# ggerganov/ggml

Measured on AMD Instinct MI355X. Metric: effective TFLOPS (2*M*N*K), Q4_K mul_mat [4096x4096]x[4096x512], higher is better.
Workload: dtype f16; 1 GPU; Q4_K MUL_MAT [4096x4096]·[4096x512] per GPU; step = Q8_K activation quantize + fp16-MFMA GEMM, W and fp32 X resident in HBM; M_per_gpu=4096, K=4096, B=512, parallelism=row-split x1, output left sharded, gemm_variant=0, splitk=0

## Files before the change

### ggml_amd/csrc/gemm_kq_t64.inc

```
#include "epilogue.h"
#include "quantize_dev.h"
template <int TYPE, int TM, bool IDS = false, int ABL = 0, bool TAIL = false, bool FQ = false>
__global__ __launch_bounds__(512) void k_gemm_kq_t64(const gemm_params p) {
    static_assert(TYPE == CDNA4_Q4_K || TYPE == CDNA4_Q4_0R, "k_gemm_kq_t64: Q4_K, and Q4_0 as its resident Q4_0R image");
    static_assert(!(FQ && TYPE != CDNA4_Q4_K), "the one-launch step quantizes to Q8_K: Q4_K only");
    static_assert(TM == 128 || TM == 256, "tile rows");
    static_assert(!(FQ && IDS), "the one-launch step is the plain MUL_MAT's");
    constexpr int TB = 128, NST = 3, BNF = 4;
    constexpr int MG = TM / 64, KW = 8 / MG;
    constexpr int NKK = 8 / KW;
    constexpr int NSB = KW == 4 ? 1 : 2;
    constexpr int RS = 256, XS = TB * RS;
    constexpr int WRS = 64, WS = TM * WRS;
    constexpr int ST = XS + WS;
    constexpr int XL = XS / 1024 / 4;
    constexpr int WL = WS / 1024 / 4;
    constexpr int NL = XL + WL;
    constexpr int BLK = QT<TYPE>::BYTES;
    constexpr int HB = TM * 16;
    constexpr int HR = TM / 4;
    constexpr int RING = NST * ST > 128 * 1024 ? NST * ST : 128 * 1024;
    constexpr int abl = ABL;
    constexpr int TRB = (ABL & 256) ? 8 * 16 * 4 * 4 : 0;
    constexpr int SMEM = RING + 2 * HB + TRB;
    static_assert(SMEM <= 160 * 1024, "LDS budget");
    __shared__ __attribute__((aligned(16))) uint8_t smem[SMEM];
    __shared__ int xchg_failed;

    const int tid = threadIdx.x, lane = tid & 63, j = lane & 31, h = lane >> 5;
    const int wave = __builtin_amdgcn_readfirstlane(tid >> 6);
    const int mg = wave % MG, kq = wave / MG;
    const int nblk = gridDim.x;
    int L = blockIdx.x;
    if ((nblk & 7) == 0 && !(IDS && p.tile_order != nullptr)) L = (blockIdx.x & 7) * (nblk >> 3) + (blockIdx.x >> 3);
    int tile_b = L % p.tiles_b, ks, tile_m;
    [[maybe_unused]] int nfrag = BNF;
    if (IDS && p.tile_order != nullptr) {
        tile_b = p.tile_order[L / p.tiles_m]; tile_m = L % p.tiles_m; ks = 0;
        nfrag = p.tile_nfrag[tile_b];
    } else { L /= p.tiles_b; ks = L % p.splitk; tile_m = L / p.splitk; }
    const int m0 = tile_m * TM, b0 = tile_b * TB;
    int64_t wexp = 0;
    if constexpr (IDS) {
        const int e = p.tile_expert[tile_b];
        if (e < 0) return;
        wexp = (int64_t)e * p.w_expert_bytes;
    }
    const int nsb_all = p.K / 256;
    int nsb, sb0;
    const bool deep = p.splitk > 2 || (p.splitk == 2 && (p.tune & 2));
    if (deep) { const int base = nsb_all / p.splitk, rem = nsb_all % p.splitk; nsb = base + (ks < rem ? 1 : 0); sb0 = ks * base + min(ks, rem); }
    else { nsb = p.partial ? (ks == 0 ? p.sb_split : nsb_all - p.sb_split) : nsb_all; sb0 = p.partial ? (ks == 0 ? 0 : p.sb_split) : 0; }
    const int nstage = nsb * 2;
    const uint32_t lds0 = CDNA4_LDS_BASE(smem);
    const bool traced = (ABL & 256) && p.trace != nullptr && blockIdx.x == 0;
    if (traced && tid == 0) { p.trace[0] = __builtin_amdgcn_s_memtime(); p.trace[1] = __builtin_amdgcn_s_memrealtime(); }
    auto mile = [&](int idx) __attribute__((always_inline)) {
        if constexpr ((ABL & 256) != 0) { if (traced && tid == 0) p.trace[idx] = __builtin_amdgcn_s_memrealtime(); }
    };
    auto stamp = [&](int s_, int ph) __attribute__((always_inline)) {
        if constexpr ((ABL & 256) != 0) {
            if (traced && s_ >= 16 && s_ < 32) {
                const uint32_t t = (uint32_t)__builtin_amdgcn_s_memtime();
                if (lane == 0) *reinterpret_cast<uint32_t *>(smem + RING + 2 * HB + ((wave * 16 + (s_ - 16)) * 4 + ph) * 4) = t;
            }
        }
    };

    floatx16 acc[2][BNF];
#pragma unroll
    for (int mb = 0; mb < 2; mb++)
#pragma unroll
        for (int i = 0; i < BNF; i++)
#pragma unroll
            for (int r = 0; r < 16; r++) acc[mb][i][r] = 0.f;

    const bool loader = wave < 4;
    uint32_t xvoff0, wvoff[WL];
    { const int pc = (wave & 3) * 64 + lane, row = pc >> 4, c = (pc & 15) ^ (row & 15); xvoff0 = (uint32_t)row * 256u + c * 16; }
#pragma unroll
    for (int i = 0; i < WL; i++) {
        const int pc = ((wave & 3) + 4 * i) * 64 + lane, row = pc >> 2, c = (pc & 3) ^ ((row >> 2) & 3);
        wvoff[i] = (uint32_t)(min(m0 + row, p.M - 1) - m0) * (uint32_t)p.w_row_bytes + c * 16;
    }
    const char *const xbase = (const char *)p.xh + ((int64_t)sb0 * 2 * p.B + b0) * 256;
    const char *const wbase = (const char *)p.W + wexp + (int64_t)m0 * p.w_row_bytes + (int64_t)sb0 * BLK + 16;
    auto issue_piece = [&](int i, int st, int slot) __attribute__((always_inline)) {
        const uint32_t l = lds0 + slot * ST;
        if (i < XL) {
            if (!(abl & 1)) {
                if constexpr (FQ) CDNA4_DMA16_SC1(xvoff0, xbase + (int64_t)st * p.B * 256 + i * 4096, l + ((wave & 3) + 4 * i) * 1024);
                else CDNA4_DMA16(xvoff0, xbase + (int64_t)st * p.B * 256 + i * 4096, l + ((wave & 3) + 4 * i) * 1024);
            }
        }
        else if (!(abl & 2)) CDNA4_DMA16(wvoff[i - XL], wbase + (int64_t)(st >> 1) * BLK + (st & 1) * 64, l + XS + ((wave & 3) + 4 * (i - XL)) * 1024);
    };
    auto issue = [&](int st, int slot) __attribute__((always_inline)) {
#pragma unroll
        for (int i = 0; i < NL; i++) issue_piece(i, st, slot);
    };
    const uint32_t hvoff = (uint32_t)(min(m0 + (wave & 3) * HR + (lane & (HR - 1)), p.M - 1) - m0) * (uint32_t)p.w_row_bytes;
    const char *const hbase = (const char *)p.W + wexp + (int64_t)m0 * p.w_row_bytes + (int64_t)sb0 * BLK;
    auto hissue = [&](int sb) __attribute__((always_inline)) {
        if (!(abl & 2)) CDNA4_DMA16_LANES(hvoff, hbase + (int64_t)sb * BLK, lds0 + RING + (sb & 1) * HB + (wave & 3) * HR * 16, HR);
    };
    auto hread = [&](int sb) __attribute__((always_inline)) { return *reinterpret_cast<const u32x4 *>(smem + RING + (sb & 1) * HB + (mg * 64 + lane) * 16); };

    DqConst dq; dq.init();
    const int gl = KW == 4 ? (kq >> 1) : kq;
    const int hi = KW == 4 ? (kq & 1) : 0;
    const int q3 = 2 * gl + hi;
    uint32_t rmask = hi ? dq.m4c : dq.m4, rmagic = hi ? dq.magic64 : dq.magic;
    const half_t roff_h = hi ? (half_t)-72.f : (half_t)-1032.f;
    const half2_t roff = {roff_h, roff_h};
    const int xswz = j & 15;

    auto sc_pack = [&](const u32x4 &hdr, auto PART, int q) __attribute__((always_inline)) -> uint32_t {
        constexpr int part = decltype(PART)::value;
        if constexpr (TYPE == CDNA4_Q4_0R) {
            const uint32_t w2 = (q >> 1) ? (part ? hdr.w : hdr.y) : (part ? hdr.z : hdr.x);
            return (w2 >> (16u * (uint32_t)(q & 1))) & 0xFFFFu;
        }
        const uint32_t sh8 = 8u * (uint32_t)q;
        uint32_t s6, m6;
        if constexpr (part == 0) { s6 = (hdr.y >> sh8) & 63u; m6 = (hdr.z >> sh8) & 63u; }
        else { s6 = ((hdr.w >> sh8) & 0xFu) | (((hdr.y >> (sh8 + 6)) & 3u) << 4); m6 = ((hdr.w >> (sh8 + 4)) & 0xFu) | (((hdr.z >> (sh8 + 6)) & 3u) << 4); }
        const float d = h2f(hdr.x & 0xFFFF), dmin = h2f(hdr.x >> 16);
        const half_t s = (half_t)(d * (float)s6);
        const half_t c = (half_t)(8.f * (float)s - dmin * (float)m6);
        return __builtin_bit_cast(uint32_t, half2_t{s, c});
    };
    Raw<TYPE> raw[2];
    typename Raw<TYPE>::Sc z[2];
    uint32_t zp[2][NSB];
    half8_t xa[2][BNF];
    uint32_t wf[2][2][4];
    if constexpr ((ABL & 4) != 0) {
#pragma unroll
        for (int i = 0; i < 2 * BNF; i++) { u32x4 zz = {(uint32_t)lane, 1u, 2u, 3u}; asm volatile("" : "+v"(zz)); xa[i / BNF][i % BNF] = __builtin_bit_cast(half8_t, zz); }
    }
    auto read_xa = [&](int slot, int set, int t, auto PF) __attribute__((always_inline)) {
        constexpr bool pf = decltype(PF)::value;
        const uint8_t *xs = smem + slot * ST + j * RS;
        const int ch = KW == 4 ? hi * 4 + 2 * h + t : (t >> 1) * 4 + 2 * h + (t & 1);
        const int coff = ((gl * 8 + ch) ^ xswz) << 4;
        if (abl & 4) return;
#pragma unroll
        for (int bf = 0; bf < BNF; bf++) if (!pf || bf < nfrag) xa[set][bf] = *reinterpret_cast<const half8_t *>(xs + bf * 32 * RS + coff);
    };
    auto read_w = [&](int slot) __attribute__((always_inline)) {
#pragma unroll
        for (int mb = 0; mb < 2; mb++) {
            const int row = mg * 64 + mb * 32 + j;
            raw[mb].q = *reinterpret_cast<const u32x4 *>(smem + slot * ST + XS + row * WRS + (((2 * gl + h) ^ ((row >> 2) & 3)) << 4));
        }
    };
    auto scales_next = [&](const u32x4 &hdr, auto PART) __attribute__((always_inline)) {
#pragma unroll
        for (int i = 0; i < NSB; i++) {
            uint32_t a = sc_pack(hdr, PART, q3 + i), b = a;
            CDNA4_SWAP32(a, b);
            zp[0][i] = a; zp[1][i] = b;
        }
    };
    auto set_z = [&]() __attribute__((always_inline)) {
#pragma unroll
        for (int mb = 0; mb < 2; mb++) {
            const half2_t lo = as_h2(zp[mb][0]);
            z[mb].SL = half2_t{lo.x, lo.x}; z[mb].CL = half2_t{lo.y, lo.y};
            if constexpr (NSB == 2) { const half2_t hh = as_h2(zp[mb][1]); z[mb].SH = half2_t{hh.x, hh.x}; z[mb].CH = half2_t{hh.y, hh.y}; }
        }
    };
    auto pbits = [&](int mb, int t, int i) __attribute__((always_inline)) -> uint32_t {
        if (abl & 8) return raw[mb].q.x;
        if constexpr (KW == 4) {
            const uint32_t src = (i < 2) ? (t ? raw[mb].q.z : raw[mb].q.x) : (t ? raw[mb].q.w : raw[mb].q.y);
            const uint32_t v = (((i & 1) ? src >> 8 : src) & rmask) | rmagic;
            const half2_t r = __builtin_elementwise_fma(as_h2(v) + roff, z[mb].SL, z[mb].CL);
            return __builtin_bit_cast(uint32_t, r);
        } else return raw[mb].pairbits(t, i, z[mb], dq);
    };
    auto mfma8 = [&](int set, auto PF, auto &&between) __attribute__((always_inline)) {
        constexpr bool pf = decltype(PF)::value;
#pragma unroll
        for (int mb = 0; mb < 2; mb++) {
            const u32x4 cw = {wf[set][mb][0], wf[set][mb][1], wf[set][mb][2], wf[set][mb][3]};
            const half8_t wfk = __builtin_bit_cast(half8_t, cw);
#pragma unroll
            for (int bf = 0; bf < BNF; bf++) {
                __builtin_amdgcn_sched_barrier(0);
                if constexpr ((ABL & 32) != 0) asm volatile("" ::"v"(xa[set][bf]), "v"(wfk));
                else if (!pf || bf < nfrag) acc[mb][bf] = __builtin_amdgcn_mfma_f32_32x32x16_f16(xa[set][bf], wfk, acc[mb][bf], 0, 0, 0);
                __builtin_amdgcn_sched_barrier(0);
                between(mb * 4 + bf);
            }
        }
    };
    typedef std::integral_constant<bool, true> yes_t; typedef std::integral_constant<bool, false> no_t;
    typedef std::integral_constant<int, 0> p0_t; typedef std::integral_constant<int, 1> p1_t;

    if constexpr (FQ) {
        const int nsbK = p.K >> 8, units = (p.tune & 8) ? 0 : p.B * nsbK, g16 = tid >> 4, l16 = tid & 15;
        int u = (int)blockIdx.x * 32 + g16;
        float e[16];
        auto load_unit = [&](int uu) __attribute__((always_inline)) {
            const int b = uu / nsbK, sb = uu - b * nsbK;
            const float *px = p.xf + (int64_t)b * p.xf_row + sb * 256 + 8 * l16;
#pragma unroll
            for (int i = 0; i < 4; i++) {
                const float4 v = *reinterpret_cast<const float4 *>(px + 128 * (i >> 1) + 4 * (i & 1));
                e[4 * i] = v.x; e[4 * i + 1] = v.y; e[4 * i + 2] = v.z; e[4 * i + 3] = v.w;
            }
        };
#pragma unroll
        for (int i = 0; i < 16; i++) e[i] = 0.f;
        if (u < units) load_unit(u);
#pragma unroll
        for (int i = 0; i < 16; i++) CDNA4_PIN(e[i]);
        if (loader) {
            hissue(0); hissue(nsb > 1 ? 1 : 0);
#pragma unroll
            for (int i = XL; i < NL; i++) issue_piece(i, 0, 0);
#pragma unroll
            for (int i = XL; i < NL; i++) issue_piece(i, 1, 1);
        }
        {
            __amdgpu_buffer_rsrc_t img = __builtin_amdgcn_make_buffer_rsrc((void *)p.xh, 0, (int)((int64_t)p.B * p.K * 2), 0x00020000);
            while (u < units) {
                const int b = u / nsbK, sb = u - b * nsbK;
                u32x4 o0, o1;
                q8_K_group16_image(e, l16, o0, o1);
                const int off0 = ((2 * sb) * p.B + b) * 256 + 16 * l16;
                __builtin_amdgcn_raw_buffer_store_b128(o0, img, off0, 0, 16);
                __builtin_amdgcn_raw_buffer_store_b128(o1, img, off0 + p.B * 256, 0, 16);
                u += nblk * 32;
                if (u < units) load_unit(u);
            }
        }
        CDNA4_WAIT_VM(0);
        __syncthreads();
        mile(4);
        if (tid == 0) {
            xchg_failed = ((p.tune & 4) || cdna4_grid_barrier(p.gbar, (unsigned)nblk)) ? 0 : 1;
            if (xchg_failed) cdna4_report_fault(p.fault, 1u);
        }
        __syncthreads();
        if (xchg_failed) {
            for (int i = tid; i < TB * TM; i += 512) {
                const int b = b0 + i / TM, m = m0 + i % TM;
                if (b < p.B && m < p.M) p.Y[(int64_t)b * p.y_row + m] = __builtin_nanf("");
            }
            return;
        }
        mile(5);
        if (loader) {
#pragma unroll
            for (int i = 0; i < XL; i++) issue_piece(i, 0, 0);
#pragma unroll
            for (int i = 0; i < XL; i++) issue_piece(i, 1, 1);
            CDNA4_WAIT_VM(XL);
        }
    } else if (loader) {
        hissue(0); hissue(nsb > 1 ? 1 : 0);
        issue(0, 0); issue(1, 1);
        CDNA4_WAIT_VM(NL);
    }
    __builtin_amdgcn_s_barrier();
    asm volatile("" ::: "memory");
    mile(6);
    u32x4 hcur = hread(0);
    read_w(0); read_xa(0, 0, 0, std::integral_constant<bool, false>{});
    scales_next(hcur, p0_t{});
    set_z();
#pragma unroll
    for (int mb = 0; mb < 2; mb++)
#pragma unroll
        for (int i = 0; i < 4; i++) wf[0][mb][i] = pbits(mb, 0, i);
    int slot = 0;
    auto stage = [&](auto LDF, auto PART, auto NXF, auto L2F, auto L3F, auto PF, int s) __attribute__((always_inline)) {
        constexpr int part = decltype(PART)::value;
        constexpr bool ld = decltype(LDF)::value, nx = decltype(NXF)::value, l2 = decltype(L2F)::value, l3 = decltype(L3F)::value;
        constexpr int G = (NKK - 1) * 8;
        const int slot1 = slot == 2 ? 0 : slot + 1, slot2 = slot == 0 ? 2 : slot - 1;
        stamp(s, 0);
        if constexpr (nx && part == 1) hcur = hread((s + 1) >> 1);
#pragma unroll
        for (int t = 0; t + 1 < NKK; t++) {
            read_xa(slot, (t + 1) & 1, t + 1, PF);
            mfma8(t & 1, PF, [&](int i8) __attribute__((always_inline)) {
                wf[(t + 1) & 1][i8 >> 2][i8 & 3] = pbits(i8 >> 2, t + 1, i8 & 3);
                if constexpr (nx) {
                    if (t == 0 && i8 == 2) { if constexpr (part == 0) scales_next(hcur, p1_t{}); else scales_next(hcur, p0_t{}); }
                }
                if constexpr (ld && l2) {
                    const int g = t * 8 + i8;
                    if constexpr (part == 1 && l3) { if (g == 0) hissue((s + 3) >> 1); }
#pragma unroll
                    for (int i = 0; i < NL; i++) if (i * G / NL == g) issue_piece(i, s + 2, slot2);
                }
            });
        }
        if constexpr (nx) {
            stamp(s, 1);
            if constexpr (ld) {
                if constexpr (l2) CDNA4_WAIT_VM(NL + ((part == 1 && l3) ? 1 : 0)); else CDNA4_WAIT_VM(0);
            }
            CDNA4_WAIT_LGKM0();
            stamp(s, 2);
            if (!(abl & 16)) __builtin_amdgcn_s_barrier();
            asm volatile("" ::: "memory");
            stamp(s, 3);
            __builtin_amdgcn_sched_barrier(0);
            read_w(slot1); read_xa(slot1, 0, 0, PF);
            __builtin_amdgcn_sched_barrier(0);
        }
        mfma8((NKK - 1) & 1, PF, [&](int i8) __attribute__((always_inline)) {
            if constexpr (nx) {
                if (i8 == 3) set_z();
                if (i8 >= 4) { const int q = (i8 - 4) * 2; wf[0][q >> 2][q & 3] = pbits(q >> 2, 0, q & 3); wf[0][(q + 1) >> 2][(q + 1) & 3] = pbits((q + 1) >> 2, 0, (q + 1) & 3); }
            }
        });
        slot = slot1;
    };
    auto k_loop = [&](auto LDF, auto PF) __attribute__((always_inline)) {
        int s = 0;
        for (; s + 5 < nstage; s += 2) { stage(LDF, p0_t{}, yes_t{}, yes_t{}, yes_t{}, PF, s); stage(LDF, p1_t{}, yes_t{}, yes_t{}, yes_t{}, PF, s + 1); }
        if (s + 3 < nstage) { stage(LDF, p0_t{}, yes_t{}, yes_t{}, yes_t{}, PF, s); stage(LDF, p1_t{}, yes_t{}, yes_t{}, no_t{}, PF, s + 1); s += 2; }
        stage(LDF, p0_t{}, yes_t{}, no_t{}, no_t{}, PF, s); stage(LDF, p1_t{}, no_t{}, no_t{}, no_t{}, PF, s + 1);
    };
    if constexpr (IDS && TM == 128) {
        if (nfrag < BNF) { if (loader) k_loop(yes_t{}, yes_t{}); else k_loop(no_t{}, yes_t{}); }
        else { if (loader) k_loop(yes_t{}, no_t{}); else k_loop(no_t{}, no_t{}); }
    } else { if (loader) k_loop(yes_t{}, no_t{}); else k_loop(no_t{}, no_t{}); }

    __syncthreads();
    if constexpr ((ABL & 256) != 0) {
        if (traced) {
            if (tid == 0) { p.trace[2] = __builtin_amdgcn_s_memtime(); p.trace[3] = __builtin_amdgcn_s_memrealtime(); }
            reinterpret_cast<uint32_t *>(p.trace + 8)[tid] = reinterpret_cast<const uint32_t *>(smem + RING + 2 * HB)[tid];
        }
    }
    float4 *red = reinterpret_cast<float4 *>(smem);
    const int tile_id = tile_m * p.tiles_b + tile_b;
    bool out_keeper = false; int out_fb0 = 0;
    constexpr bool has_tail = TAIL && !IDS;
    auto finish = [&](auto KQ) __attribute__((always_inline)) {
        constexpr int kqc = decltype(KQ)::value;
        constexpr int H1 = KW / 2;
        constexpr int keep0 = (kqc & H1) ? 2 : 0, send0 = 2 - keep0;
        float4 *mine = red + (size_t)(mg + MG * kqc) * 1024, *theirs = red + (size_t)(mg + MG * (kqc ^ H1)) * 1024;
#pragma unroll
        for (int mb = 0; mb < 2; mb++)
#pragma unroll
            for (int e = 0; e < 2; e++)
#pragma unroll
                for (int q4 = 0; q4 < 4; q4++) {
                    const floatx16 &a = acc[mb][send0 + e];
                    mine[((mb * 2 + e) * 4 + q4) * 64 + lane] = make_float4(a[4 * q4], a[4 * q4 + 1], a[4 * q4 + 2], a[4 * q4 + 3]);
                }
        __syncthreads();
#pragma unroll
        for (int mb = 0; mb < 2; mb++)
#pragma unroll
            for (int e = 0; e < 2; e++)
#pragma unroll
                for (int q4 = 0; q4 < 4; q4++) {
                    const float4 v = theirs[((mb * 2 + e) * 4 + q4) * 64 + lane];
                    floatx16 &a = acc[mb][keep0 + e];
                    a[4 * q4] += v.x; a[4 * q4 + 1] += v.y; a[4 * q4 + 2] += v.z; a[4 * q4 + 3] += v.w;
                }
        constexpr int NBH = KW == 4 ? 1 : 2;
        constexpr int fb0 = KW == 4 ? keep0 + (kqc & 1) : keep0;
        if constexpr (KW == 4) {
            constexpr int give = keep0 + 1 - (kqc & 1);
            float4 *theirs2 = red + (size_t)(mg + MG * (kqc ^ 1)) * 1024;
            __syncthreads();
#pragma unroll
            for (int mb = 0; mb < 2; mb++)
#pragma unroll
                for (int q4 = 0; q4 < 4; q4++) {
                    const floatx16 &a = acc[mb][give];
                    mine[(mb * 4 + q4) * 64 + lane] = make_float4(a[4 * q4], a[4 * q4 + 1], a[4 * q4 + 2], a[4 * q4 + 3]);
                }
            __syncthreads();
#pragma unroll
            for (int mb = 0; mb < 2; mb++)
#pragma unroll
                for (int q4 = 0; q4 < 4; q4++) {
                    const float4 v = theirs2[(mb * 4 + q4) * 64 + lane];
                    floatx16 &a = acc[mb][fb0];
                    a[4 * q4] += v.x; a[4 * q4 + 1] += v.y; a[4 * q4 + 2] += v.z; a[4 * q4 + 3] += v.w;
                }
        }
        bool keeper = true;
        if (TM == 128 && deep) {
            constexpr int WF4 = NBH * 2 * 4 * 64;
            const int S = p.splitk;
            float4 *slots = reinterpret_cast<float4 *>(p.partial) + ((size_t)tile_id * S * 8 + (mg + MG * kqc)) * WF4;
            {
                __amdgpu_buffer_rsrc_t rsrc = __builtin_amdgcn_make_buffer_rsrc(slots + (size_t)ks * 8 * WF4, 0, WF4 * 16, 0x00020000);
#pragma unroll
                for (int e = 0; e < NBH; e++)
#pragma unroll
                    for (int mb = 0; mb < 2; mb++)
#pragma unroll
                        for (int q4 = 0; q4 < 4; q4++) {
                            const floatx16 &a = acc[mb][fb0 + e];
                            const float4 v = make_float4(a[4 * q4], a[4 * q4 + 1], a[4 * q4 + 2], a[4 * q4 + 3]);
                            __builtin_amdgcn_raw_buffer_store_b128(__builtin_bit_cast(u32x4, v), rsrc, (((e * 2 + mb) * 4 + q4) * 64 + lane) * 16, 0, 16);
                        }
                CDNA4_WAIT_VM(0);
            }
            __syncthreads();
            if (tid == 0) {
                unsigned *ticket = p.flags + 8192 + tile_id;
                const unsigned old = __hip_atomic_fetch_add(ticket, 1u, __ATOMIC_RELAXED, __HIP_MEMORY_SCOPE_AGENT);
                xchg_failed = old == (unsigned)(S - 1);
                if (xchg_failed) __hip_atomic_store(ticket, 0u, __ATOMIC_RELAXED, __HIP_MEMORY_SCOPE_AGENT);
            }
            __syncthreads();
            keeper = xchg_failed != 0;
            if (keeper) {
                float4 sum[NBH * 8];
                for (int k2 = 0; k2 < S; k2++) {
                    float4 v[NBH * 8];
                    if (k2 == ks) {
#pragma unroll
                        for (int e = 0; e < NBH; e++)
#pragma unroll
                            for (int mb = 0; mb < 2; mb++)
#pragma unroll
                                for (int q4 = 0; q4 < 4; q4++) { const floatx16 &a = acc[mb][fb0 + e]; v[(e * 2 + mb) * 4 + q4] = make_float4(a[4 * q4], a[4 * q4 + 1], a[4 * q4 + 2], a[4 * q4 + 3]); }
                    } else {
                        __amdgpu_buffer_rsrc_t rin = __builtin_amdgcn_make_buffer_rsrc(slots + (size_t)k2 * 8 * WF4, 0, WF4 * 16, 0x00020000);
#pragma unroll
                        for (int i = 0; i < NBH * 8; i++) v[i] = __builtin_bit_cast(float4, __builtin_amdgcn_raw_buffer_load_b128(rin, (i * 64 + lane) * 16, 0, 17));
                    }
#pragma unroll
                    for (int i = 0; i < NBH * 8; i++) {
                        if (k2 == 0) sum[i] = v[i];
                        else { sum[i].x += v[i].x; sum[i].y += v[i].y; sum[i].z += v[i].z; sum[i].w += v[i].w; }
                    }
                }
#pragma unroll
                for (int e = 0; e < NBH; e++)
#pragma unroll
                    for (int mb = 0; mb < 2; mb++)
#pragma unroll
                        for (int q4 = 0; q4 < 4; q4++) {
                            const float4 v = sum[(e * 2 + mb) * 4 + q4];
                            floatx16 &a = acc[mb][fb0 + e];
                            a[4 * q4] = v.x; a[4 * q4 + 1] = v.y; a[4 * q4 + 2] = v.z; a[4 * q4 + 3] = v.w;
                        }
            }
        } else if (p.partial) {
            mile(266);
            constexpr int WF4 = NBH * 2 * 4 * 64;
            keeper = (fb0 >> 1) == ks;
            float4 *slot_out = reinterpret_cast<float4 *>(p.partial) + ((size_t)(tile_id * 2 + (ks ^ 1)) * 8 + (mg + MG * kqc)) * WF4;
            float4 *slot_in = reinterpret_cast<float4 *>(p.partial) + ((size_t)(tile_id * 2 + ks) * 8 + (mg + MG * kqc)) * WF4;
            const unsigned my_xcc = __builtin_amdgcn_s_getreg(20 | (3 << 11)) & 15u;
            if (!keeper) {
                __amdgpu_buffer_rsrc_t rsrc = __builtin_amdgcn_make_buffer_rsrc(slot_out, 0, WF4 * 16, 0x00020000);
#pragma unroll
                for (int e = 0; e < NBH; e++)
#pragma unroll
                    for (int mb = 0; mb < 2; mb++)
#pragma unroll
                        for (int q4 = 0; q4 < 4; q4++) {
                            const floatx16 &a = acc[mb][fb0 + e];
                            const float4 v = make_float4(a[4 * q4], a[4 * q4 + 1], a[4 * q4 + 2], a[4 * q4 + 3]);
                            const int off = (((e * 2 + mb) * 4 + q4) * 64 + lane) * 16;
                            if (p.xchg_l2) __builtin_amdgcn_raw_buffer_store_b128(__builtin_bit_cast(u32x4, v), rsrc, off, 0, 0);
                            else __builtin_amdgcn_raw_buffer_store_b128(__builtin_bit_cast(u32x4, v), rsrc, off, 0, 16);
                        }
                CDNA4_WAIT_VM(0);
            }
            __syncthreads();
            mile(267);
            if (tid == 0) {
                __hip_atomic_store(p.flags + tile_id * 2 + ks, 16u | my_xcc, __ATOMIC_RELAXED, __HIP_MEMORY_SCOPE_AGENT);
                unsigned spins = 0, v;
                while ((v = __hip_atomic_load(p.flags + tile_id * 2 + (ks ^ 1), __ATOMIC_RELAXED, __HIP_MEMORY_SCOPE_AGENT)) == 0 && ++spins < CDNA4_SPIN_BOUND) __builtin_amdgcn_s_sleep(1);
                xchg_failed = spins >= CDNA4_SPIN_BOUND || (p.xchg_l2 && (v & 15u) != my_xcc);
                if (xchg_failed) cdna4_report_fault(p.fault, 2u);
            }
            __syncthreads();
            mile(268);
            if (keeper) {
                __amdgpu_buffer_rsrc_t rin = __builtin_amdgcn_make_buffer_rsrc(slot_in, 0, WF4 * 16, 0x00020000);
                float4 o[NBH * 8];
#pragma unroll
                for (int i = 0; i < NBH * 8; i++) o[i] = __builtin_bit_cast(float4, __builtin_amdgcn_raw_buffer_load_b128(rin, (i * 64 + lane) * 16, 0, 17));
                if (xchg_failed) {
#pragma unroll
                    for (int i = 0; i < NBH * 8; i++) o[i].x = __builtin_nanf("");
                }
#pragma unroll
                for (int e = 0; e < NBH; e++)
#pragma unroll
                    for (int mb = 0; mb < 2; mb++)
#pragma unroll
                        for (int q4 = 0; q4 < 4; q4++) {
                            const float4 v = o[(e * 2 + mb) * 4 + q4];
                            floatx16 &a = acc[mb][fb0 + e];
                            a[4 * q4] += v.x; a[4 * q4 + 1] += v.y; a[4 * q4 + 2] += v.z; a[4 * q4 + 3] += v.w;
                        }
            }
            __syncthreads();
            if (tid == 0) __hip_atomic_store(p.flags + tile_id * 2 + (ks ^ 1), 0u, __ATOMIC_RELAXED, __HIP_MEMORY_SCOPE_AGENT);
        }
        out_keeper = keeper; out_fb0 = fb0;
        mile(7);
        if constexpr (!has_tail) {
            if (keeper) {
#pragma unroll
                for (int e = 0; e < NBH; e++)
#pragma unroll
                    for (int mb = 0; mb < 2; mb++) {
                        const int m = m0 + mg * 64 + mb * 32 + j;
#pragma unroll
                        for (int r = 0; r < 16; r++) {
                            const int b = b0 + (fb0 + e) * 32 + (r & 3) + 8 * (r >> 2) + 4 * h;
                            if constexpr (IDS) {
                                const int pr = b < p.B ? p.row_dst[b] : -1;
                                if (pr >= 0 && m < p.M) p.Y[(int64_t)pr * p.y_row + m] = acc[mb][fb0 + e][r];
                            } else if (b < p.B && m < p.M) p.Y[(int64_t)b * p.y_row + m] = acc[mb][fb0 + e][r];
                        }
                    }
            }
        } else {
            __syncthreads();
            if (keeper) {
#pragma unroll
                for (int e = 0; e < NBH; e++)
#pragma unroll
                    for (int mb = 0; mb < 2; mb++)
#pragma unroll
                        for (int q4 = 0; q4 < 4; q4++) {
                            const floatx16 &a = acc[mb][fb0 + e];
                            mine[((e * 2 + mb) * 4 + q4) * 64 + lane] = make_float4(a[4 * q4], a[4 * q4 + 1], a[4 * q4 + 2], a[4 * q4 + 3]);
                        }
            }
        }
    };
    if constexpr (KW == 4) {
        if (kq == 0) finish(std::integral_constant<int, 0>{}); else if (kq == 1) finish(std::integral_constant<int, 1>{});
        else if (kq == 2) finish(std::integral_constant<int, 2>{}); else finish(std::integral_constant<int, 3>{});
    } else {
        if (kq == 0) finish(std::integral_constant<int, 0>{}); else finish(std::integral_constant<int, 1>{});
    }
    if constexpr ((ABL & 256) != 0) {
        mile(265);
        if (traced) { CDNA4_WAIT_VM(0); __syncthreads(); mile(264); }
    }
    if constexpr (has_tail) if (out_keeper) {
        constexpr int NBH_ = KW == 4 ? 1 : 2;
        asm volatile("" ::: "memory");
        const float *stg = reinterpret_cast<const float *>(red + (size_t)(mg + MG * kq) * 1024);
        const bool has_bias = !IDS && p.epi.bias != nullptr, has_act = !IDS && p.epi.act == 1, has_res = !IDS && p.epi.resid != nullptr;
#pragma unroll 4
        for (int idx = 0; idx < NBH_ * 32; idx++) {
            const int e = idx >> 5, mb = (idx >> 4) & 1, r = idx & 15;
            const int m = m0 + mg * 64 + mb * 32 + j;
            const int b = b0 + (out_fb0 + e) * 32 + (r & 3) + 8 * (r >> 2) + 4 * h;
            float v = stg[((((e * 2 + mb) * 4 + (r >> 2)) * 64 + lane) << 2) + (r & 3)];
            if (b < p.B && m < p.M) {
                if (has_bias) v = v + p.epi.bias[m];
                if (has_act) v = gelu_lut_f32(v);
                if (has_res) v = v + p.epi.resid[(int64_t)b * p.epi.resid_row_stride + m];
                p.Y[(int64_t)b * p.y_row + m] = v;
            }
        }
    }
}
```

### ggml_amd/csrc/gemm_q_hw.h

```cpp
#pragma once
#ifndef CDNA4_HW_OVERRIDE
#define CDNA4_LDS_BASE(smem_) ((uint32_t)(uintptr_t)(__attribute__((address_space(3))) uint8_t *)(smem_))
#define CDNA4_DMA16(voff, sbase, lds_addr) asm volatile("s_mov_b32 m0, %2\n\ts_nop 0\n\tglobal_load_lds_dwordx4 %0, %1" ::"v"(voff), "s"(sbase), "s"(lds_addr) : "memory", "m0")
#define CDNA4_DMA16_SC1(voff, sbase, lds_addr) asm volatile("s_mov_b32 m0, %2\n\ts_nop 0\n\tglobal_load_lds_dwordx4 %0, %1 sc1" ::"v"(voff), "s"(sbase), "s"(lds_addr) : "memory", "m0")
#define CDNA4_GLOAD16_PTR(dst, ptr) asm volatile("global_load_dwordx4 %0, %1, off" : "=v"(dst) : "v"(ptr) : "memory")
#define CDNA4_WAIT_VM_TIED1(n, a) asm volatile("s_waitcnt vmcnt(%1)" : "+v"(a) : "n"(n) : "memory")
#define CDNA4_WAIT_VM_TIED2(n, a, b) asm volatile("s_waitcnt vmcnt(%2)" : "+v"(a), "+v"(b) : "n"(n) : "memory")
#define CDNA4_WAIT_VM(n) asm volatile("s_waitcnt vmcnt(%0)" ::"n"(n) : "memory")
#define CDNA4_WAIT_LGKM0() asm volatile("s_waitcnt lgkmcnt(0)" ::: "memory")
#define CDNA4_WAIT_VM_CASE(n) case n: asm volatile("s_waitcnt vmcnt(" #n ")" ::: "memory"); break;
__device__ __forceinline__ void cdna4_wait_vm_rt(int n) {
    switch (n < 0 ? 0 : (n > 24 ? 24 : n)) {
        CDNA4_WAIT_VM_CASE(0) CDNA4_WAIT_VM_CASE(1) CDNA4_WAIT_VM_CASE(2) CDNA4_WAIT_VM_CASE(3) CDNA4_WAIT_VM_CASE(4) CDNA4_WAIT_VM_CASE(5) CDNA4_WAIT_VM_CASE(6)
        CDNA4_WAIT_VM_CASE(7) CDNA4_WAIT_VM_CASE(8) CDNA4_WAIT_VM_CASE(9) CDNA4_WAIT_VM_CASE(10) CDNA4_WAIT_VM_CASE(11) CDNA4_WAIT_VM_CASE(12) CDNA4_WAIT_VM_CASE(13)
        CDNA4_WAIT_VM_CASE(14) CDNA4_WAIT_VM_CASE(15) CDNA4_WAIT_VM_CASE(16) CDNA4_WAIT_VM_CASE(17) CDNA4_WAIT_VM_CASE(18) CDNA4_WAIT_VM_CASE(19) CDNA4_WAIT_VM_CASE(20)
        CDNA4_WAIT_VM_CASE(21) CDNA4_WAIT_VM_CASE(22) CDNA4_WAIT_VM_CASE(23) CDNA4_WAIT_VM_CASE(24)
    }
}
#define CDNA4_PIN(x) asm volatile("" : "+v"(x))
#define CDNA4_WAIT_LGKM0_VISIBLE() do { __builtin_amdgcn_s_waitcnt(0xC07F); asm volatile("" ::: "memory"); } while (0)
#define CDNA4_DMA16_LANES(voff, sbase, lds_addr, nlanes) do { uint64_t cdna4_exec_;                                                   \
    asm volatile("s_mov_b64 %0, exec\n\ts_mov_b64 exec, %4\n\ts_mov_b32 m0, %3\n\ts_nop 0\n\tglobal_load_lds_dwordx4 %1, %2\n\ts_mov_b64 exec, %0" \
                 : "=&s"(cdna4_exec_) : "v"(voff), "s"(sbase), "s"(lds_addr), "i"((nlanes) >= 64 ? -1ll : (long long)((1ull << ((nlanes) & 63)) - 1)) : "memory", "m0"); } while (0)
#define CDNA4_SWAP32(a, b) do { auto r_ = __builtin_amdgcn_permlane32_swap((a), (b), false, false); (a) = r_[0]; (b) = r_[1]; } while (0)
#endif
```

Baseline: 538.9 TFLOP/s.

## Replace templated per-kq epilogue dispatch with runtime-selected reduction and strided stores

The cross-wave K reduction epilogue was a lambda instantiated once per kq value and selected by a runtime branch chain. It is now one runtime code path that parks and takes accumulator halves through LDS into a separate fin array. This shrinks code size and may lower register pressure. The non-IDS full-tile output store now walks a precomputed byte pointer with fixed row strides and skips the per-element bounds checks, and a new scalar pin macro keeps the stride in SGPRs. The risk is runtime selects on acc fragments, which can add VGPR moves or force spills.

```diff
diff --git a/ggml_amd/csrc/gemm_kq_t64.inc b/ggml_amd/csrc/gemm_kq_t64.inc
--- a/ggml_amd/csrc/gemm_kq_t64.inc
+++ b/ggml_amd/csrc/gemm_kq_t64.inc
@@ -342,61 +342,60 @@
     }
     float4 *red = reinterpret_cast<float4 *>(smem);
     const int tile_id = tile_m * p.tiles_b + tile_b;
-    bool out_keeper = false; int out_fb0 = 0;
     constexpr bool has_tail = TAIL && !IDS;
-    auto finish = [&](auto KQ) __attribute__((always_inline)) {
-        constexpr int kqc = decltype(KQ)::value;
-        constexpr int H1 = KW / 2;
-        constexpr int keep0 = (kqc & H1) ? 2 : 0, send0 = 2 - keep0;
-        float4 *mine = red + (size_t)(mg + MG * kqc) * 1024, *theirs = red + (size_t)(mg + MG * (kqc ^ H1)) * 1024;
-#pragma unroll
-        for (int mb = 0; mb < 2; mb++)
-#pragma unroll
-            for (int e = 0; e < 2; e++)
-#pragma unroll
-                for (int q4 = 0; q4 < 4; q4++) {
-                    const floatx16 &a = acc[mb][send0 + e];
-                    mine[((mb * 2 + e) * 4 + q4) * 64 + lane] = make_float4(a[4 * q4], a[4 * q4 + 1], a[4 * q4 + 2], a[4 * q4 + 3]);
-                }
-        __syncthreads();
-#pragma unroll
-        for (int mb = 0; mb < 2; mb++)
-#pragma unroll
-            for (int e = 0; e < 2; e++)
-#pragma unroll
-                for (int q4 = 0; q4 < 4; q4++) {
-                    const float4 v = theirs[((mb * 2 + e) * 4 + q4) * 64 + lane];
-                    floatx16 &a = acc[mb][keep0 + e];
-                    a[4 * q4] += v.x; a[4 * q4 + 1] += v.y; a[4 * q4 + 2] += v.z; a[4 * q4 + 3] += v.w;
-                }
-        constexpr int NBH = KW == 4 ? 1 : 2;
-        constexpr int fb0 = KW == 4 ? keep0 + (kqc & 1) : keep0;
+    constexpr int H1 = KW / 2;
+    constexpr int NBH = KW == 4 ? 1 : 2;
+    const bool upper = (kq & H1) != 0;
+    const int fb0 = KW == 4 ? kq : (upper ? 2 : 0);
+    float4 *mine = red + (size_t)(mg + MG * kq) * 1024, *theirs = red + (size_t)(mg + MG * (kq ^ H1)) * 1024;
+    float fin[NBH][2][16];
+    int tl = lane;
+    CDNA4_PIN(tl);
+    const int tj = tl & 31, th = tl >> 5;
+    auto park = [&](const auto &x0, const auto &x1, int slot, int nslot) __attribute__((always_inline)) {
+#pragma unroll
+        for (int q4 = 0; q4 < 4; q4++) {
+            mine[((0 * nslot + slot) * 4 + q4) * 64 + tl] = make_float4(x0[4 * q4], x0[4 * q4 + 1], x0[4 * q4 + 2], x0[4 * q4 + 3]);
+            mine[((1 * nslot + slot) * 4 + q4) * 64 + tl] = make_float4(x1[4 * q4], x1[4 * q4 + 1], x1[4 * q4 + 2], x1[4 * q4 + 3]);
+        }
+    };
+    auto take = [&](const auto &x0, const auto &x1, float (&o0)[16], float (&o1)[16], const float4 *from, int slot, int nslot) __attribute__((always_inline)) {
+#pragma unroll
+        for (int q4 = 0; q4 < 4; q4++) {
+            const float4 v = from[((0 * nslot + slot) * 4 + q4) * 64 + tl], w = from[((1 * nslot + slot) * 4 + q4) * 64 + tl];
+            o0[4 * q4] = x0[4 * q4] + v.x; o0[4 * q4 + 1] = x0[4 * q4 + 1] + v.y; o0[4 * q4 + 2] = x0[4 * q4 + 2] + v.z; o0[4 * q4 + 3] = x0[4 * q4 + 3] + v.w;
+            o1[4 * q4] = x1[4 * q4] + w.x; o1[4 * q4 + 1] = x1[4 * q4 + 1] + w.y; o1[4 * q4 + 2] = x1[4 * q4 + 2] + w.z; o1[4 * q4 + 3] = x1[4 * q4 + 3] + w.w;
+        }
+    };
+    bool keeper = true;
+    {
         if constexpr (KW == 4) {
-            constexpr int give = keep0 + 1 - (kqc & 1);
-            float4 *theirs2 = red + (size_t)(mg + MG * (kqc ^ 1)) * 1024;
-            __syncthreads();
-#pragma unroll
-            for (int mb = 0; mb < 2; mb++)
-#pragma unroll
-                for (int q4 = 0; q4 < 4; q4++) {
-                    const floatx16 &a = acc[mb][give];
-                    mine[(mb * 4 + q4) * 64 + lane] = make_float4(a[4 * q4], a[4 * q4 + 1], a[4 * q4 + 2], a[4 * q4 + 3]);
-                }
-            __syncthreads();
-#pragma unroll
-            for (int mb = 0; mb < 2; mb++)
-#pragma unroll
-                for (int q4 = 0; q4 < 4; q4++) {
-                    const float4 v = theirs2[(mb * 4 + q4) * 64 + lane];
-                    floatx16 &a = acc[mb][fb0];
-                    a[4 * q4] += v.x; a[4 * q4 + 1] += v.y; a[4 * q4 + 2] += v.z; a[4 * q4 + 3] += v.w;
-                }
-        }
-        bool keeper = true;
+            float mid[2][2][16];
+            if (upper) { park(acc[0][0], acc[1][0], 0, 2); park(acc[0][1], acc[1][1], 1, 2); } else { park(acc[0][2], acc[1][2], 0, 2); park(acc[0][3], acc[1][3], 1, 2); }
+            __syncthreads();
+            if (upper) { take(acc[0][2], acc[1][2], mid[0][0], mid[0][1], theirs, 0, 2); take(acc[0][3], acc[1][3], mid[1][0], mid[1][1], theirs, 1, 2); }
+            else { take(acc[0][0], acc[1][0], mid[0][0], mid[0][1], theirs, 0, 2); take(acc[0][1], acc[1][1], mid[1][0], mid[1][1], theirs, 1, 2); }
+            const float4 *theirs2 = red + (size_t)(mg + MG * (kq ^ 1)) * 1024;
+            const bool odd = (kq & 1) != 0;
+            __syncthreads();
+            if (odd) park(mid[0][0], mid[0][1], 0, 1); else park(mid[1][0], mid[1][1], 0, 1);
+            __syncthreads();
+            if (odd) take(mid[1][0], mid[1][1], fin[0][0], fin[0][1], theirs2, 0, 1); else take(mid[0][0], mid[0][1], fin[0][0], fin[0][1], theirs2, 0, 1);
+        } else {
+            if (upper) {
+#pragma unroll
+                for (int mb = 0; mb < 2; mb++)
+#pragma unroll
+                    for (int e = 0; e < 2; e++) { const floatx16 t = acc[mb][e]; acc[mb][e] = acc[mb][e + 2]; acc[mb][e + 2] = t; }
+            }
+            park(acc[0][2], acc[1][2], 0, 2); park(acc[0][3], acc[1][3], 1, 2);
+            __syncthreads();
+            take(acc[0][0], acc[1][0], fin[0][0], fin[0][1], theirs, 0, 2); take(acc[0][1], acc[1][1], fin[NBH - 1][0], fin[NBH - 1][1], theirs, 1, 2);
+        }
         if (TM == 128 && deep) {
             constexpr int WF4 = NBH * 2 * 4 * 64;
             const int S = p.splitk;
-            float4 *slots = reinterpret_cast<float4 *>(p.partial) + ((size_t)tile_id * S * 8 + (mg + MG * kqc)) * WF4;
+            float4 *slots = reinterpret_cast<float4 *>(p.partial) + ((size_t)tile_id * S * 8 + (mg + MG * kq)) * WF4;
             {
                 __amdgpu_buffer_rsrc_t rsrc = __builtin_amdgcn_make_buffer_rsrc(slots + (size_t)ks * 8 * WF4, 0, WF4 * 16, 0x00020000);
 #pragma unroll
@@ -405,9 +404,9 @@
                     for (int mb = 0; mb < 2; mb++)
 #pragma unroll
                         for (int q4 = 0; q4 < 4; q4++) {
-                            const floatx16 &a = acc[mb][fb0 + e];
+                            const float *a = fin[e][mb];
                             const float4 v = make_float4(a[4 * q4], a[4 * q4 + 1], a[4 * q4 + 2], a[4 * q4 + 3]);
-                            __builtin_amdgcn_raw_buffer_store_b128(__builtin_bit_cast(u32x4, v), rsrc, (((e * 2 + mb) * 4 + q4) * 64 + lane) * 16, 0, 16);
+                            __builtin_amdgcn_raw_buffer_store_b128(__builtin_bit_cast(u32x4, v), rsrc, (((e * 2 + mb) * 4 + q4) * 64 + tl) * 16, 0, 16);
                         }
                 CDNA4_WAIT_VM(0);
             }
@@ -430,11 +429,11 @@
 #pragma unroll
                             for (int mb = 0; mb < 2; mb++)
 #pragma unroll
-                                for (int q4 = 0; q4 < 4; q4++) { const floatx16 &a = acc[mb][fb0 + e]; v[(e * 2 + mb) * 4 + q4] = make_float4(a[4 * q4], a[4 * q4 + 1], a[4 * q4 + 2], a[4 * q4 + 3]); }
+                                for (int q4 = 0; q4 < 4; q4++) { const float *a = fin[e][mb]; v[(e * 2 + mb) * 4 + q4] = make_float4(a[4 * q4], a[4 * q4 + 1], a[4 * q4 + 2], a[4 * q4 + 3]); }
                     } else {
                         __amdgpu_buffer_rsrc_t rin = __builtin_amdgcn_make_buffer_rsrc(slots + (size_t)k2 * 8 * WF4, 0, WF4 * 16, 0x00020000);
 #pragma unroll
-                        for (int i = 0; i < NBH * 8; i++) v[i] = __builtin_bit_cast(float4, __builtin_amdgcn_raw_buffer_load_b128(rin, (i * 64 + lane) * 16, 0, 17));
+                        for (int i = 0; i < NBH * 8; i++) v[i] = __builtin_bit_cast(float4, __builtin_amdgcn_raw_buffer_load_b128(rin, (i * 64 + tl) * 16, 0, 17));
                     }
 #pragma unroll
                     for (int i = 0; i < NBH * 8; i++) {
@@ -449,7 +448,7 @@
 #pragma unroll
                         for (int q4 = 0; q4 < 4; q4++) {
                             const float4 v = sum[(e * 2 + mb) * 4 + q4];
-                            floatx16 &a = acc[mb][fb0 + e];
+                            float *a = fin[e][mb];
                             a[4 * q4] = v.x; a[4 * q4 + 1] = v.y; a[4 * q4 + 2] = v.z; a[4 * q4 + 3] = v.w;
                         }
             }
@@ -457,8 +456,8 @@
             mile(266);
             constexpr int WF4 = NBH * 2 * 4 * 64;
             keeper = (fb0 >> 1) == ks;
-            float4 *slot_out = reinterpret_cast<float4 *>(p.partial) + ((size_t)(tile_id * 2 + (ks ^ 1)) * 8 + (mg + MG * kqc)) * WF4;
-            float4 *slot_in = reinterpret_cast<float4 *>(p.partial) + ((size_t)(tile_id * 2 + ks) * 8 + (mg + MG * kqc)) * WF4;
+            float4 *slot_out = reinterpret_cast<float4 *>(p.partial) + ((size_t)(tile_id * 2 + (ks ^ 1)) * 8 + (mg + MG * kq)) * WF4;
+            float4 *slot_in = reinterpret_cast<float4 *>(p.partial) + ((size_t)(tile_id * 2 + ks) * 8 + (mg + MG * kq)) * WF4;
             const unsigned my_xcc = __builtin_amdgcn_s_getreg(20 | (3 << 11)) & 15u;
             if (!keeper) {
                 __amdgpu_buffer_rsrc_t rsrc = __builtin_amdgcn_make_buffer_rsrc(slot_out, 0, WF4 * 16, 0x00020000);
@@ -468,9 +467,9 @@
                     for (int mb = 0; mb < 2; mb++)
 #pragma unroll
                         for (int q4 = 0; q4 < 4; q4++) {
-                            const floatx16 &a = acc[mb][fb0 + e];
+                            const float *a = fin[e][mb];
                             const float4 v = make_float4(a[4 * q4], a[4 * q4 + 1], a[4 * q4 + 2], a[4 * q4 + 3]);
-                            const int off = (((e * 2 + mb) * 4 + q4) * 64 + lane) * 16;
+                            const int off = (((e * 2 + mb) * 4 + q4) * 64 + tl) * 16;
                             if (p.xchg_l2) __builtin_amdgcn_raw_buffer_store_b128(__builtin_bit_cast(u32x4, v), rsrc, off, 0, 0);
                             else __builtin_amdgcn_raw_buffer_store_b128(__builtin_bit_cast(u32x4, v), rsrc, off, 0, 16);
                         }
@@ -491,7 +490,7 @@
                 __amdgpu_buffer_rsrc_t rin = __builtin_amdgcn_make_buffer_rsrc(slot_in, 0, WF4 * 16, 0x00020000);
                 float4 o[NBH * 8];
 #pragma unroll
-                for (int i = 0; i < NBH * 8; i++) o[i] = __builtin_bit_cast(float4, __builtin_amdgcn_raw_buffer_load_b128(rin, (i * 64 + lane) * 16, 0, 17));
+                for (int i = 0; i < NBH * 8; i++) o[i] = __builtin_bit_cast(float4, __builtin_amdgcn_raw_buffer_load_b128(rin, (i * 64 + tl) * 16, 0, 17));
                 if (xchg_failed) {
 #pragma unroll
                     for (int i = 0; i < NBH * 8; i++) o[i].x = __builtin_nanf("");
@@ -503,67 +502,89 @@
 #pragma unroll
                         for (int q4 = 0; q4 < 4; q4++) {
                             const float4 v = o[(e * 2 + mb) * 4 + q4];
-                            floatx16 &a = acc[mb][fb0 + e];
+                            float *a = fin[e][mb];
                             a[4 * q4] += v.x; a[4 * q4 + 1] += v.y; a[4 * q4 + 2] += v.z; a[4 * q4 + 3] += v.w;
                         }
             }
             __syncthreads();
             if (tid == 0) __hip_atomic_store(p.flags + tile_id * 2 + (ks ^ 1), 0u, __ATOMIC_RELAXED, __HIP_MEMORY_SCOPE_AGENT);
         }
-        out_keeper = keeper; out_fb0 = fb0;
         mile(7);
         if constexpr (!has_tail) {
             if (keeper) {
+                if constexpr (IDS || KW == 2) {
+#pragma unroll
+                    for (int e = 0; e < NBH; e++)
+#pragma unroll
+                        for (int mb = 0; mb < 2; mb++) {
+                            const int m = m0 + mg * 64 + mb * 32 + tj;
+#pragma unroll
+                            for (int r = 0; r < 16; r++) {
+                                const int b = b0 + (fb0 + e) * 32 + (r & 3) + 8 * (r >> 2) + 4 * th;
+                                if constexpr (IDS) {
+                                    const int pr = b < p.B ? p.row_dst[b] : -1;
+                                    if (pr >= 0 && m < p.M) p.Y[(int64_t)pr * p.y_row + m] = fin[e][mb][r];
+                                } else if (b < p.B && m < p.M) p.Y[(int64_t)b * p.y_row + m] = fin[e][mb][r];
+                            }
+                        }
+                } else {
+                    const int64_t rstep = p.y_row * 4;
+                    int64_t rstep5 = rstep * 5;
+                    CDNA4_PIN_S64(rstep5);
+                    char *row = reinterpret_cast<char *>(p.Y + ((int64_t)(b0 + fb0 * 32) * p.y_row + (m0 + mg * 64)))
+                                + ((th ? rstep * 4 : (int64_t)0) + tj * 4);
+                    if (b0 + TB <= p.B && m0 + TM <= p.M) {
+#pragma unroll
+                        for (int e = 0; e < NBH; e++)
+#pragma unroll
+                            for (int r = 0; r < 16; r++) {
+#pragma unroll
+                                for (int mb = 0; mb < 2; mb++) *reinterpret_cast<float *>(row + mb * 128) = fin[e][mb][r];
+                                row += (r & 3) == 3 ? rstep5 : rstep;
+                            }
+                    } else {
+                        const int nb = p.B - (b0 + fb0 * 32) - 4 * th;
+                        const bool mok[2] = {m0 + mg * 64 + tj < p.M, m0 + mg * 64 + 32 + tj < p.M};
+#pragma unroll
+                        for (int e = 0; e < NBH; e++)
+#pragma unroll
+                            for (int r = 0; r < 16; r++) {
+                                const int dr = e * 32 + (r & 3) + 8 * (r >> 2);
+#pragma unroll
+                                for (int mb = 0; mb < 2; mb++) if (mok[mb] && dr < nb) *reinterpret_cast<float *>(row + mb * 128) = fin[e][mb][r];
+                                row += (r & 3) == 3 ? rstep5 : rstep;
+                            }
+                    }
+                }
+            }
+        } else {
+            __syncthreads();
+            if (keeper) {
 #pragma unroll
                 for (int e = 0; e < NBH; e++)
 #pragma unroll
-                    for (int mb = 0; mb < 2; mb++) {
-                        const int m = m0 + mg * 64 + mb * 32 + j;
-#pragma unroll
-                        for (int r = 0; r < 16; r++) {
-                            const int b = b0 + (fb0 + e) * 32 + (r & 3) + 8 * (r >> 2) + 4 * h;
-                            if constexpr (IDS) {
-                                const int pr = b < p.B ? p.row_dst[b] : -1;
-                                if (pr >= 0 && m < p.M) p.Y[(int64_t)pr * p.y_row + m] = acc[mb][fb0 + e][r];
-                            } else if (b < p.B && m < p.M) p.Y[(int64_t)b * p.y_row + m] = acc[mb][fb0 + e][r];
+                    for (int mb = 0; mb < 2; mb++)
+#pragma unroll
+                        for (int q4 = 0; q4 < 4; q4++) {
+                            const float *a = fin[e][mb];
+                            mine[((e * 2 + mb) * 4 + q4) * 64 + tl] = make_float4(a[4 * q4], a[4 * q4 + 1], a[4 * q4 + 2], a[4 * q4 + 3]);
                         }
-                    }
-            }
-        } else {
-            __syncthreads();
-            if (keeper) {
-#pragma unroll
-                for (int e = 0; e < NBH; e++)
-#pragma unroll
-                    for (int mb = 0; mb < 2; mb++)
-#pragma unroll
-                        for (int q4 = 0; q4 < 4; q4++) {
-                            const floatx16 &a = acc[mb][fb0 + e];
-                            mine[((e * 2 + mb) * 4 + q4) * 64 + lane] = make_float4(a[4 * q4], a[4 * q4 + 1], a[4 * q4 + 2], a[4 * q4 + 3]);
-                        }
-            }
-        }
-    };
-    if constexpr (KW == 4) {
-        if (kq == 0) finish(std::integral_constant<int, 0>{}); else if (kq == 1) finish(std::integral_constant<int, 1>{});
-        else if (kq == 2) finish(std::integral_constant<int, 2>{}); else finish(std::integral_constant<int, 3>{});
-    } else {
-        if (kq == 0) finish(std::integral_constant<int, 0>{}); else finish(std::integral_constant<int, 1>{});
+            }
+        }
     }
     if constexpr ((ABL & 256) != 0) {
         mile(265);
         if (traced) { CDNA4_WAIT_VM(0); __syncthreads(); mile(264); }
     }
-    if constexpr (has_tail) if (out_keeper) {
-        constexpr int NBH_ = KW == 4 ? 1 : 2;
+    if constexpr (has_tail) if (keeper) {
         asm volatile("" ::: "memory");
         const float *stg = reinterpret_cast<const float *>(red + (size_t)(mg + MG * kq) * 1024);
         const bool has_bias = !IDS && p.epi.bias != nullptr, has_act = !IDS && p.epi.act == 1, has_res = !IDS && p.epi.resid != nullptr;
 #pragma unroll 4
-        for (int idx = 0; idx < NBH_ * 32; idx++) {
+        for (int idx = 0; idx < NBH * 32; idx++) {
             const int e = idx >> 5, mb = (idx >> 4) & 1, r = idx & 15;
             const int m = m0 + mg * 64 + mb * 32 + j;
-            const int b = b0 + (out_fb0 + e) * 32 + (r & 3) + 8 * (r >> 2) + 4 * h;
+            const int b = b0 + (fb0 + e) * 32 + (r & 3) + 8 * (r >> 2) + 4 * h;
             float v = stg[((((e * 2 + mb) * 4 + (r >> 2)) * 64 + lane) << 2) + (r & 3)];
             if (b < p.B && m < p.M) {
                 if (has_bias) v = v + p.epi.bias[m];
diff --git a/ggml_amd/csrc/gemm_q_hw.h b/ggml_amd/csrc/gemm_q_hw.h
--- a/ggml_amd/csrc/gemm_q_hw.h
+++ b/ggml_amd/csrc/gemm_q_hw.h
@@ -18,6 +18,7 @@
     }
 }
 #define CDNA4_PIN(x) asm volatile("" : "+v"(x))
+#define CDNA4_PIN_S64(x) asm volatile("" : "+s"(x))
 #define CDNA4_WAIT_LGKM0_VISIBLE() do { __builtin_amdgcn_s_waitcnt(0xC07F); asm volatile("" ::: "memory"); } while (0)
 #define CDNA4_DMA16_LANES(voff, sbase, lds_addr, nlanes) do { uint64_t cdna4_exec_;                                                   \
     asm volatile("s_mov_b64 %0, exec\n\ts_mov_b64 exec, %4\n\ts_mov_b32 m0, %3\n\ts_nop 0\n\tglobal_load_lds_dwordx4 %1, %2\n\ts_mov_b64 exec, %0" \
```

Measured after the change: 535.7 TFLOP/s. About the same (-0.6%).
